# alan-turing-institute/mogp-emulator

Measured on AMD Instinct MI355X. Metric: GP fits/sec (+ fit+grad/s, predict pts/s), 64-output n=2000 d=10 on 1 MI355X, fp64, higher is better.
Workload: dtype f64

## Files before the change

### mogp_emulator_amd/csrc/kernels_mchol.hip

```cpp
#include <algorithm>
#include <cmath>
#include <cstdio>
#include <cstdlib>
#include <utility>
#include <vector>
#define MOGP_OPAQUE_TID 1
#include "launch.h"
#include "chol128_dev.h"
#include "trsm_dev.h"
#include "gemm_dev.h"

namespace mogp {

namespace {

constexpr int MC_LINE = 32;
constexpr int MC_ABORT = 0, MC_TIMEOUTS = 1;
constexpr int MC_HEADS = MC_LINE;
constexpr int MC_EMU0 = MC_LINE * 9;
constexpr int MC_AHEAD_BIT = 1 << 29;
constexpr int MC_PD = 4;
constexpr int MC_LDS_HDR = 4;

__device__ __forceinline__ unsigned ldu(const unsigned* p) { return __hip_atomic_load(p, __ATOMIC_RELAXED, __HIP_MEMORY_SCOPE_AGENT); }
__device__ __forceinline__ void stu(unsigned* p, unsigned x) { __hip_atomic_store(p, x, __ATOMIC_RELAXED, __HIP_MEMORY_SCOPE_AGENT); }
__device__ __forceinline__ void drain_stores() { asm volatile("s_waitcnt vmcnt(0)" ::: "memory"); }

#ifndef MOGP_MC_SCHED
#define MOGP_MC_SCHED 3
#endif
constexpr int MC_SCHED = MOGP_MC_SCHED;
template <int BM, int BN>
__device__ __forceinline__ void MC_GEMM(const double* __restrict__ Ag, int lda, const double* __restrict__ Bg, int ldb, int nk, v4d (&acc)[BM / 32][BN / 32],
                                        double* smem, int kmask) {
  mainloop_q<BM, BN, 2, 2, 2, MC_SCHED>(Ag, lda, Bg, ldb, nk, acc, smem, kmask);
}
constexpr size_t MC_GEMM_LDS = QCfg<64, 128>::SMEM_DOUBLES;

struct McCtx {
  unsigned* ctrl;
  int spin_limit;
  int* shi;
};

constexpr int MC_TRW = 30;
template <bool TRACE>
__device__ __forceinline__ void mc_stamp(unsigned long long* tr, int i) {
  if (TRACE && tr && threadIdx.x == 0) tr[i] = __builtin_amdgcn_s_memrealtime();
}

__device__ __forceinline__ int mc_wait_min4(const McCtx& cx, const unsigned* a, const unsigned* b, const unsigned* c, const unsigned* d, unsigned want,
                                            unsigned long long* waited = nullptr) {
  if (threadIdx.x == 0) {
    const unsigned long long w0 = waited ? __builtin_amdgcn_s_memrealtime() : 0ull;
    int res, spins = 0;
    for (;;) {
      unsigned m = ldu(a);
      const unsigned mb = ldu(b), mc = ldu(c), md = ldu(d);
      m = m < mb ? m : mb;
      m = m < mc ? m : mc;
      m = m < md ? m : md;
      if (m >= want) {
        res = (int)m;
        break;
      }
      ++spins;
      if (spins > cx.spin_limit) {
        stu(cx.ctrl + MC_ABORT, 1u);
        __hip_atomic_fetch_add(cx.ctrl + MC_TIMEOUTS, 1u, __ATOMIC_RELAXED, __HIP_MEMORY_SCOPE_AGENT);
        res = -1;
        break;
      }
      if ((spins & 31) == 0 && ldu(cx.ctrl + MC_ABORT) != 0u) {
        res = -1;
        break;
      }
      __builtin_amdgcn_s_sleep(1);
    }
    cx.shi[1] = res;
    if (waited) waited[9] += __builtin_amdgcn_s_memrealtime() - w0;
  }
  __syncthreads();
  const int r = cx.shi[1];
  __syncthreads();
  return r;
}

__device__ __forceinline__ int mc_wait_min3(const McCtx& cx, const unsigned* a, const unsigned* b, const unsigned* c, unsigned want,
                                            unsigned long long* waited = nullptr) {
  return mc_wait_min4(cx, a, b, c, c, want, waited);
}

struct PieceWait {
  const McCtx& cx;
  const unsigned *a, *b;
  unsigned base;
  int avail;
  unsigned long long* tr;
  __device__ __forceinline__ bool known(int j) const { return avail > j; }
  __device__ __forceinline__ bool operator()(int j) {
    if (avail > j) return true;
    const int m = mc_wait_min3(cx, a, b, b, base + (unsigned)j + 1u, tr);
    if (m < 0) return false;
    avail = m - (int)base;
    return true;
  }
};

}

template <bool TRACE, bool SOLO = false>
__global__ __launch_bounds__(256, SOLO ? 1 : 2) void mchol_kernel(BatchView v, unsigned* __restrict__ ctrl, const int* __restrict__ table, int ntasks,
                                                       int emu_stride, double* __restrict__ packs, int* __restrict__ info, int nq, int spin_limit,
                                                       unsigned long long* __restrict__ trace, int opts) {
  extern __shared__ __attribute__((aligned(16))) double smem[];
  int* shi = reinterpret_cast<int*>(smem);
  double* lds = smem + MC_LDS_HDR;
  McCtx cx{ctrl, spin_limit, shi};
  const int t = threadIdx.x;
  const int ld = v.LD;
  const int K = v.NP / 128, K2 = v.NP / 64;
  const int home = (int)blockIdx.x & (nq - 1);
  const int emus_q = v.nb / nq;
  const int total = ntasks * emus_q;
  const int gs = ((opts >> 12) & 0xff) ? ((opts >> 12) & 0xff) : emus_q;
  for (int qi = 0; qi < nq; ++qi) {
    const int q = (home + qi) & (nq - 1);
    unsigned* head = ctrl + MC_HEADS + q * MC_LINE;
    int next_tk = -1;
    auto draw_next = [&]() {
      if (t == 0 && next_tk < 0) next_tk = (int)__hip_atomic_fetch_add(head, 1u, __ATOMIC_RELAXED, __HIP_MEMORY_SCOPE_AGENT);
    };
    for (;;) {
      draw_next();
      if (t == 0) shi[0] = next_tk;
      __syncthreads();
      const int tk = shi[0];
      __syncthreads();
      if (tk >= total) break;
      next_tk = -1;
      const int per = ntasks * gs, grp = tk / per, rem = tk - grp * per;
      const int p = rem / gs, zl = grp * gs + (rem - p * gs);
      const int z = zl * nq + q;
      const int emu = __builtin_amdgcn_readfirstlane(v.idx ? v.idx[z] : z);
      const int word = table[p];
      const int type = (word >> 30) & 3, c = (word >> 15) & 0x3fff, r = word & 0x7fff;
      const bool listed_ahead = (word & MC_AHEAD_BIT) != 0;
      double* A = v.A + (size_t)emu * v.MS;
      unsigned* rowdone = ctrl + MC_EMU0 + (size_t)z * emu_stride;
      unsigned* diagcnt = rowdone + K2;
      unsigned* ddone = diagcnt + K;
      unsigned* rowprog = ddone + K;
      double* pk = packs + ((size_t)z * K + c) * PACK128_STRIDE;
      const int c0 = 128 * c;
      unsigned long long* tr = TRACE ? trace + ((size_t)z * ntasks + p) * MC_TRW : nullptr;
      if (TRACE && t == 0) {
        tr[6] = __builtin_amdgcn_s_getreg(6164) | ((unsigned long long)__builtin_amdgcn_s_getreg(((8 - 1) << 11) | (8 << 6) | 4) << 8);
        tr[7] = (unsigned)word | ((unsigned long long)tk << 32);
      }
      mc_stamp<TRACE>(tr, 0);
      if (type == 0) {
        mc_stamp<TRACE>(tr, 1);
        if (c > 1 && mc_wait_min3(cx, diagcnt + c, diagcnt + c, diagcnt + c, 3u, tr) < 0) return;
        auto inputs_seen = [&]() { mc_stamp<TRACE>(tr, 2); };
        if (c > 0) {
          PieceWait pw{cx, rowprog + 2 * c, rowprog + 2 * c + 1, 8u * (unsigned)(c - 1), 0, tr};
          if (!chol128_dev<true, true, true>(A + (size_t)c0 * ld + c0, ld, pk, info + emu, c0, lds, ddone + c, pw, inputs_seen)) return;
        } else {
          inputs_seen();
          chol128_dev<true, false, true>(A + (size_t)c0 * ld + c0, ld, pk, info + emu, c0, lds, ddone + c);
        }
        __builtin_amdgcn_s_setprio(0);
        drain_stores();
        __syncthreads();
        if (t == 0) stu(ddone + c, 8u);
        mc_stamp<TRACE>(tr, 5);
        continue;
      }
      if (type == 1) {
        const int ti = r > 0 ? 1 : 0, tj = r > 1 ? 1 : 0;
        const int gi0 = c0 + 64 * ti, gj0 = c0 + 64 * tj;
        __builtin_amdgcn_s_setprio(2);
        v4d acc[2][2];
        double* pcG = A + (size_t)(gi0 + (t >> 7) * 32 + ((t & 63) >> 4)) * ld + (gj0 + ((t >> 6) & 1) * 32 + (t & 15));
#pragma unroll
        for (int i = 0; i < 2; ++i)
#pragma unroll
          for (int j = 0; j < 2; ++j)
#pragma unroll
            for (int q = 0; q < 4; ++q) acc[i][j][q] = SOLO ? -pcG[(size_t)(i * 16 + 4 * q) * ld + j * 16] : 0.0;
        const int kend = c - 1;
        int kb = 0;
        while (kb < kend) {
          mc_stamp<TRACE>(tr, 1);
          int m = mc_wait_min3(cx, rowdone + 2 * c + ti, rowdone + 2 * c + tj, rowdone + 2 * c + tj, (unsigned)(kb + 1), tr);
          if (m < 0) return;
          mc_stamp<TRACE>(tr, 2);
          m = m < kend ? m : kend;
          MC_GEMM<64, 64>(A + (size_t)gi0 * ld + 128 * kb, ld, A + (size_t)gj0 * ld + 128 * kb, ld, 8 * (m - kb), acc, lds, -1);
          kb = m;
        }
        mc_stamp<TRACE>(tr, 3);
        draw_next();
        {
          double cv[2][2][4];
          if (!SOLO) {
#pragma unroll
            for (int i = 0; i < 2; ++i)
#pragma unroll
              for (int j = 0; j < 2; ++j)
#pragma unroll
                for (int q = 0; q < 4; ++q) cv[i][j][q] = pcG[(size_t)(i * 16 + 4 * q) * ld + j * 16];
          }
#pragma unroll
          for (int i = 0; i < 2; ++i)
#pragma unroll
            for (int j = 0; j < 2; ++j)
#pragma unroll
              for (int q = 0; q < 4; ++q)
                __hip_atomic_store(pcG + (size_t)(i * 16 + 4 * q) * ld + j * 16, SOLO ? -acc[i][j][q] : cv[i][j][q] - acc[i][j][q], __ATOMIC_RELAXED,
                                   __HIP_MEMORY_SCOPE_AGENT);
        }
        drain_stores();
        mc_stamp<TRACE>(tr, 4);
        __syncthreads();
        if (t == 0) __hip_atomic_fetch_add(diagcnt + c, 1u, __ATOMIC_RELAXED, __HIP_MEMORY_SCOPE_AGENT);
        mc_stamp<TRACE>(tr, 5);
        __builtin_amdgcn_s_setprio(0);
        continue;
      }
      const int r0 = 64 * r;
      const bool urgent = r < 2 * c + 4 + 2 * ((opts >> 8) & 3);
      if (urgent) __builtin_amdgcn_s_setprio(2);
      const int kend = c;
      if (kend > 0) {
        v4d acc[2][4];
        const double* pcT = A + (size_t)(r0 + (t >> 7) * 32 + ((t & 63) >> 4)) * ld + (c0 + ((t >> 6) & 1) * 64 + (t & 15));
#pragma unroll
        for (int i = 0; i < 2; ++i)
#pragma unroll
          for (int j = 0; j < 4; ++j)
#pragma unroll
            for (int q = 0; q < 4; ++q) acc[i][j][q] = SOLO ? -pcT[(size_t)(i * 16 + 4 * q) * ld + j * 16] : 0.0;
        auto finish_x = [&]() {
          if (SOLO) {
#pragma unroll
            for (int i = 0; i < 2; ++i)
#pragma unroll
              for (int j = 0; j < 4; ++j) acc[i][j] = -acc[i][j];
          } else {
            double cv[2][4][4];
#pragma unroll
            for (int i = 0; i < 2; ++i)
#pragma unroll
              for (int j = 0; j < 4; ++j)
#pragma unroll
                for (int q = 0; q < 4; ++q) cv[i][j][q] = pcT[(size_t)(i * 16 + 4 * q) * ld + j * 16];
#pragma unroll
            for (int i = 0; i < 2; ++i)
#pragma unroll
              for (int j = 0; j < 4; ++j)
#pragma unroll
                for (int q = 0; q < 4; ++q) acc[i][j][q] = cv[i][j][q] - acc[i][j][q];
          }
        };
        {
          int ks = 0;
          const int kse = 8 * kend;
          while (ks < kse) {
            mc_stamp<TRACE>(tr, 1);
            int have = mc_wait_min3(cx, rowprog + r, rowprog + 2 * c, rowprog + 2 * c + 1, (unsigned)(ks + MC_PD), tr);
            if (have < 0) return;
            mc_stamp<TRACE>(tr, 2);
            have = (have < kse ? have : kse) & ~(MC_PD - 1);
            MC_GEMM<64, 128>(A + (size_t)r0 * ld + 16 * ks, ld, A + (size_t)c0 * ld + 16 * ks, ld, have - ks, acc, lds,
                             (opts & 2) ? 3 : -1);
            ks = have;
          }
        }
        mc_stamp<TRACE>(tr, 3);
        if (!listed_ahead) draw_next();
        if (!urgent) {
          if (mc_wait_min3(cx, ddone + c, ddone + c, ddone + c, 8u, tr) < 0) return;
          TrsmSlabPre SP;
          trsm128_slab_request(pk, SP);
          finish_x();
          mc_stamp<TRACE>(tr, 4);
          mc_stamp<TRACE>(tr, 8);
          __builtin_amdgcn_s_setprio(1);
          trsm128_tile2_dev<true>(v, c0, r0, pk, emu, lds, acc, SP, TRACE ? tr + 10 : nullptr);
          drain_stores();
          mc_stamp<TRACE>(tr, 13);
          __syncthreads();
          if (t == 0) {
            stu(rowprog + r, 8u * (unsigned)(c + 1));
            stu(rowdone + r, (unsigned)(c + 1));
          }
          mc_stamp<TRACE>(tr, 5);
          __builtin_amdgcn_s_setprio(0);
          continue;
        }
        {
          finish_x();
          mc_stamp<TRACE>(tr, 4);
          bool first = true;
          auto wait = [&](int b) {
            const bool ok = mc_wait_min3(cx, ddone + c, ddone + c, ddone + c, (unsigned)(b + 1), tr) >= 0;
            if (first) mc_stamp<TRACE>(tr, 8);
            first = false;
            return ok;
          };
          auto pub = [&](int b) {
            if (t == 0) stu(rowprog + r, 8u * (unsigned)c + (unsigned)b + 1u);
          };
          const int prog = mc_wait_min3(cx, ddone + c, ddone + c, ddone + c, 0u);
          if (prog < 0) return;
          if (prog >= 8) {
            mc_stamp<TRACE>(tr, 8);
            trsm128_tile2_chain_dev<true, true>(v, c0, r0, pk, emu, lds, acc, TrsmNoWait(), pub);
          } else if (!trsm128_tile2_chain_dev<true, false>(v, c0, r0, pk, emu, lds, acc, wait, pub)) return;
          drain_stores();
          __syncthreads();
          if (t == 0) {
            stu(rowprog + r, 8u * (unsigned)(c + 1));
            stu(rowdone + r, (unsigned)(c + 1));
          }
          mc_stamp<TRACE>(tr, 5);
          __builtin_amdgcn_s_setprio(0);
          continue;
        }
      }
      if (urgent) {
        bool first = true;
        auto wait = [&](int b) {
          const bool ok = mc_wait_min3(cx, ddone + c, ddone + c, ddone + c, (unsigned)(b + 1), tr) >= 0;
          if (first) mc_stamp<TRACE>(tr, 8);
          first = false;
          return ok;
        };
        auto pub = [&](int b) {
          if (t == 0) stu(rowprog + r, 8u * (unsigned)c + (unsigned)b + 1u);
        };
        const int prog = mc_wait_min3(cx, ddone + c, ddone + c, ddone + c, 0u);
        if (prog < 0) return;
        if (prog >= 8) {
          mc_stamp<TRACE>(tr, 8);
          trsm128_lds_dev<true, true, false>(v, c0, r0, pk, emu, 0, lds, TrsmNoWait(), pub);
        } else if (!trsm128_lds_dev<true, false, true>(v, c0, r0, pk, emu, 0, lds, wait, pub)) return;
      } else {
        if (mc_wait_min3(cx, ddone + c, ddone + c, ddone + c, 8u, tr) < 0) return;
        mc_stamp<TRACE>(tr, 8);
        __builtin_amdgcn_s_setprio(1);
        trsm128_lds_dev<true, true>(v, c0, r0, pk, emu, 0, lds);
      }
      drain_stores();
      __syncthreads();
      if (t == 0) {
        stu(rowprog + r, 8u * (unsigned)(c + 1));
        stu(rowdone + r, (unsigned)(c + 1));
      }
      mc_stamp<TRACE>(tr, 5);
      __builtin_amdgcn_s_setprio(0);
    }
  }
}

std::vector<int> mchol_task_table(int NP, bool ahead) {
  const int K = NP / 128, K2 = NP / 64;
  auto word = [](int type, int c, int r) { return (int)(((unsigned)type << 30) | ((unsigned)c << 15) | (unsigned)r); };
  std::vector<std::pair<long, int>> keyed;
  const long M = 4L * K2 + 64;
  long slot = 0;
  int iter = -1;
  auto put = [&](int w, bool band) {
    const bool moved = band && ahead && iter >= 1;
    keyed.push_back({(long)((moved ? iter - 1 : iter) + 1) * M + (moved ? M / 2 : 0) + slot, moved ? (w | MC_AHEAD_BIT) : w});
    ++slot;
  };
  auto T = [&](int r, int c, bool band) {
    if (c < K && r < K2 && r >= 2 * c + 2) put(word(2, c, r), band);
  };
  put(word(0, 0, 0), false);
  T(2, 0, false);
  T(3, 0, false);
  T(4, 0, false);
  T(5, 0, false);
  for (int c = 0; c < K; ++c) {
    iter = c;
    slot = 0;
    if (c + 1 < K) put(word(0, c + 1, 0), false);
    T(2 * c + 4, c + 1, true);
    T(2 * c + 5, c + 1, true);
    if (c + 2 < K)
      for (int sub = 0; sub < 3; ++sub) put(word(1, c + 2, sub), false);
    T(2 * c + 6, c, true);
    T(2 * c + 7, c, true);
    T(2 * c + 6, c + 1, true);
    T(2 * c + 7, c + 1, true);
    for (int r = 2 * c + 8; r < K2; ++r) T(r, c, false);
  }
  std::stable_sort(keyed.begin(), keyed.end(), [](const std::pair<long, int>& a, const std::pair<long, int>& b) { return a.first < b.first; });
  std::vector<int> tb;
  for (auto& kw : keyed) tb.push_back(kw.second);
  return tb;
}

int mchol_emu_stride(int NP) { return (2 * (NP / 64) + 2 * (NP / 128) + MC_LINE - 1) / MC_LINE * MC_LINE; }
size_t mchol_ctrl_ints(int NP, int B) { return MC_EMU0 + (size_t)B * mchol_emu_stride(NP); }
size_t mchol_pack_doubles(int NP, int B) { return (size_t)B * (NP / 128) * PACK128_STRIDE; }

static double mchol_rho(int nb, int NP) {
  const double npd = NP;
  return ((double)nb * npd * npd * npd / 3.0 / 45e12) / ((npd / 128.0) * 55e-6);
}

void launch_mchol(const BatchView& v, unsigned* ctrl, size_t ctrl_ints, const int* tables, int ntasks, double* packs, int* info, int n_cu,
                  hipStream_t s, bool ctrl_zeroed) {
  static const int spin_limit = [] { const char* e = getenv("MOGP_MC_SPIN"); return e ? atoi(e) : (1 << 22); }();
  const double rho = mchol_rho(v.nb, v.NP);
  const double K16 = std::max(1.0, (v.NP / 128) / 16.0);
  const int per_cu = rho < 1.2 * std::pow(K16, 0.7) ? 1 : 2;

  if (!ctrl_zeroed) (void)hipMemsetAsync(ctrl, 0, ctrl_ints * sizeof(unsigned), s);
  const int nq = (v.nb % 8 == 0) ? 8 : 1;
  const size_t lds_need = MC_LDS_HDR + std::max<size_t>({(size_t)MC_GEMM_LDS, (size_t)TRSM128L_LDS, (size_t)C128_LDS_PRE_DOUBLES, (size_t)TRSM128T_LDS});
  const size_t lds_doubles = per_cu == 1 ? std::max<size_t>(lds_need, 10 * 1024 + 64) : lds_need;
  const int total = ntasks * v.nb;
  const int grid = std::min(per_cu * n_cu, total);
  const bool ahead = rho >= 0.2 && rho < 2.0 && 8 * (v.nb / nq) <= grid / nq;
  const int* table = tables + (ahead ? ntasks : 0);
  static const char* trace_file = getenv("MOGP_MC_TRACE");
  const size_t words = (size_t)total * MC_TRW;
  unsigned long long* dtr = nullptr;
  const int emus_q = v.nb / nq, wg_q = std::max(1, grid / nq);
  int gsz = 0;
  if (v.NP >= 2048)
    for (int g = 1; g < emus_q; ++g)
      if (emus_q % g == 0 && 4 * g * (v.NP / 64) >= 5 * wg_q) {
        gsz = g;
        break;
      }
  const int opts = ((rho < 1.0 ? 2 : 0) << 8) | (gsz << 12);
  if (trace_file) {
    if (hipMalloc(reinterpret_cast<void**>(&dtr), words * 8) != hipSuccess) {
      dtr = nullptr;
      fprintf(stderr, "libmogp_hip: MOGP_MC_TRACE: no device memory for %zu stamp words, this factorisation is not traced\n", words);
    }
  }
  if (trace_file && dtr) {
    (void)hipMemsetAsync(dtr, 0, words * 8, s);
    hipLaunchKernelGGL(mchol_kernel<true>, dim3(grid), dim3(256), lds_doubles * sizeof(double), s, v, ctrl, table, ntasks, mchol_emu_stride(v.NP), packs,
                       info, nq, spin_limit, dtr, opts);
    std::vector<unsigned long long> h(words);
    (void)hipStreamSynchronize(s);
    (void)hipMemcpy(h.data(), dtr, words * 8, hipMemcpyDeviceToHost);
    (void)hipFree(dtr);
    if (FILE* f = fopen(trace_file, "ab")) {
      const long long hdr[4] = {v.nb, ntasks, v.NP, grid + 1000000LL * MC_TRW};
      fwrite(hdr, sizeof(hdr), 1, f);
      fwrite(h.data(), 8, words, f);
      fclose(f);
    }
    return;
  }
  prof_begin("mchol", s);
  if (per_cu == 1)
    hipLaunchKernelGGL((mchol_kernel<false, true>), dim3(grid), dim3(256), lds_doubles * sizeof(double), s, v, ctrl, table, ntasks, mchol_emu_stride(v.NP), packs,
                     info, nq, spin_limit, (unsigned long long*)nullptr, opts);
  else
    hipLaunchKernelGGL(mchol_kernel<false>, dim3(grid), dim3(256), lds_doubles * sizeof(double), s, v, ctrl, table, ntasks, mchol_emu_stride(v.NP), packs,
                     info, nq, spin_limit, (unsigned long long*)nullptr, opts);
  const double n = v.n;
  prof_end("mchol", s, (double)v.nb * n * n * n / 3.0, (double)v.nb * 8.0 * n * n);
}

}
```

### mogp_emulator_amd/csrc/trsm_dev.h

```cpp
#pragma once
#include <type_traits>
#include "launch.h"
#include "chol128_dev.h"

namespace mogp {

typedef double v4d_t __attribute__((ext_vector_type(4)));
typedef double v2d_p __attribute__((ext_vector_type(2)));

constexpr int TL_PK = 112 * 16 + 256;
constexpr int TL_TS = 16 * 18;
constexpr int TRSM128L_LDS = 2 * TL_PK + 4 * 2 * TL_TS;

struct TrsmNoWait {
  __device__ __forceinline__ bool operator()(int) const { return true; }
};
struct TrsmNoPub {
  __device__ __forceinline__ void operator()(int) const {}
};
template <bool SC1_OUT = false, bool DEEP = false, bool PIPE = false, class WAIT = TrsmNoWait, class PUB = TrsmNoPub>
__device__ __forceinline__ bool trsm128_lds_dev(const BatchView& v, int c0, int r0, const double* __restrict__ pk, int emu, int rowblock,
                                                double* lds, WAIT wait = WAIT(), PUB pub = PUB()) {
  constexpr bool PUBLISH = (PIPE || DEEP) && !std::is_same<PUB, TrsmNoPub>::value;
  Sc1Buf ab;
  if (SC1_OUT) ab = sc1_buf(v.A + (size_t)emu * v.MS, (unsigned)(v.MS * sizeof(double)));
  const int ld = v.LD;
  const int t = mogp_tid(), lane = t & 63, wave = __builtin_amdgcn_readfirstlane(t >> 6);
  const int g = lane >> 4, i = lane & 15;
  double* slab = v.A + (size_t)emu * v.MS + (size_t)(r0 + rowblock * 64 + wave * 16) * ld + c0;
  double* pkb[2] = {lds, lds + TL_PK};
  double* tsb[2] = {lds + 2 * TL_PK + wave * 2 * TL_TS, lds + 2 * TL_PK + wave * 2 * TL_TS + TL_TS};
  const double* LT = pk + PACK128_LT;
  const int sr0 = lane >> 3, sp = (lane & 7) * 2;
  constexpr bool PRE_SLAB = DEEP || PIPE;
  v2d_p sl[PRE_SLAB ? 8 : 1][2];
  auto slab_request = [&](int b) {
    sl[PRE_SLAB ? b : 0][0] = *reinterpret_cast<const v2d_p*>(slab + (size_t)sr0 * ld + 16 * b + sp);
    sl[PRE_SLAB ? b : 0][1] = *reinterpret_cast<const v2d_p*>(slab + (size_t)(sr0 + 8) * ld + 16 * b + sp);
  };
  auto slab_deposit = [&](int b, double* ts) {
    *reinterpret_cast<v2d_p*>(ts + sr0 * 18 + sp) = sl[PRE_SLAB ? b : 0][0];
    *reinterpret_cast<v2d_p*>(ts + (sr0 + 8) * 18 + sp) = sl[PRE_SLAB ? b : 0][1];
  };
  v2d_p pr[DEEP ? 2 : 1][4], pinv[DEEP ? 2 : 1];
  auto pack_request = [&](int b) {
    const int u = DEEP ? (b & 1) : 0;
#pragma unroll
    for (int q = 0; q < 4; ++q) {
      const int ch = t + 256 * q;
      if (ch < 128 * b) pr[u][q] = *reinterpret_cast<const v2d_p*>(LT + (size_t)(ch >> 3) * 128 + 16 * b + (ch & 7) * 2);
    }
    if (t < 128) pinv[u] = *reinterpret_cast<const v2d_p*>(pk + PACK128_INV + b * 256 + 2 * t);
  };
  auto pack_deposit = [&](int b, double* img) {
    const int u = DEEP ? (b & 1) : 0;
#pragma unroll
    for (int q = 0; q < 4; ++q) {
      const int ch = t + 256 * q;
      if (ch < 128 * b) *reinterpret_cast<v2d_p*>(img + (ch >> 3) * 16 + (ch & 7) * 2) = pr[u][q];
    }
    if (t < 128) *reinterpret_cast<v2d_p*>(img + 112 * 16 + 2 * t) = pinv[u];
  };
  if (PIPE) {
#pragma unroll
    for (int b = 0; b < 8; ++b) slab_request(b);
    if (!wait(0)) return false;
    pack_request(0);
  } else {
    pack_request(0);
    if (DEEP) {
      pack_request(1);
#pragma unroll
      for (int b = 0; b < 8; ++b) slab_request(b);
    } else {
      slab_request(0);
    }
  }
  pack_deposit(0, pkb[0]);
  slab_deposit(0, tsb[0]);
  __syncthreads();
  v4d_t X[8];
#pragma unroll
  for (int b = 0; b < 8; ++b) {
    const double* img = pkb[b & 1];
    double* ts = tsb[b & 1];
    if (PIPE) {
    } else if (DEEP) {
      if (b + 2 < 8) pack_request(b + 2);
    } else if (b < 7) {
      pack_request(b + 1);
      slab_request(b + 1);
    }
    v4d_t T;
#pragma unroll
    for (int r = 0; r < 4; ++r) T[r] = ts[i * 18 + g + 4 * r];
#pragma unroll
    for (int a = 0; a < b; ++a)
#pragma unroll
      for (int r = 0; r < 4; ++r)
        T = __builtin_amdgcn_mfma_f64_16x16x4f64(-img[(16 * a + g + 4 * r) * 16 + i], X[a][r], T, 0, 0, 0);
    const double* inv = img + 112 * 16;
    X[b] = (v4d_t){0., 0., 0., 0.};
#pragma unroll
    for (int r = 0; r < 4; ++r) X[b] = __builtin_amdgcn_mfma_f64_16x16x4f64(inv[(g + 4 * r) * 16 + i], T[r], X[b], 0, 0, 0);
#pragma unroll
    for (int r = 0; r < 4; ++r) ts[i * 18 + g + 4 * r] = X[b][r];
    __builtin_amdgcn_wave_barrier();
    {
      const v2d_p o0 = *reinterpret_cast<const v2d_p*>(ts + sr0 * 18 + sp);
      const v2d_p o1 = *reinterpret_cast<const v2d_p*>(ts + (sr0 + 8) * 18 + sp);
      st16<SC1_OUT>(ab, slab + (size_t)sr0 * ld + 16 * b + sp, o0);
      st16<SC1_OUT>(ab, slab + (size_t)(sr0 + 8) * ld + 16 * b + sp, o1);
    }
    if (PUBLISH && b < 7) {
      asm volatile("s_waitcnt vmcnt(0)" ::: "memory");
      __syncthreads();
      pub(b);
    }
    if (b < 7) {
      if (PIPE) {
        if (!wait(b + 1)) return false;
        pack_request(b + 1);
      }
      pack_deposit(b + 1, pkb[(b + 1) & 1]);
      slab_deposit(b + 1, tsb[(b + 1) & 1]);
    }
    __syncthreads();
  }
  return true;
}

constexpr int TRSM128T_LDS = 2 * TL_PK + 16 * TL_TS;
struct TrsmSlabPre {
  v2d_p pr[2][4], pinv[2];
};
__device__ __forceinline__ void trsm128_slab_request(const double* __restrict__ pk, TrsmSlabPre& P) {
  const int t = mogp_tid();
  const double* LT = pk + PACK128_LT;
#pragma unroll
  for (int b = 0; b < 2; ++b) {
#pragma unroll
    for (int q = 0; q < 4; ++q) {
      const int ch = t + 256 * q;
      if (ch < 128 * (7 - b)) P.pr[b][q] = *reinterpret_cast<const v2d_p*>(LT + (size_t)(16 * b + ((ch >> 3) & 15)) * 128 + 16 * (b + 1 + (ch >> 7)) + (ch & 7) * 2);
    }
    if (t < 128) P.pinv[b] = *reinterpret_cast<const v2d_p*>(pk + PACK128_INV + b * 256 + 2 * t);
  }
}

constexpr int TL_TS17 = 16 * 17;
static_assert(32 * TL_TS17 <= TRSM128T_LDS, "whole-tile stage must fit the LDS of the half-tile form");
template <bool SC1_OUT>
__device__ __forceinline__ void trsm128_tile2_dev(const BatchView& v, int c0, int r0, const double* __restrict__ pk, int emu, double* lds,
                                                  const v4d_t (&x)[2][4], TrsmSlabPre& P, unsigned long long* stamps = nullptr) {
  Sc1Buf ab;
  if (SC1_OUT) ab = sc1_buf(v.A + (size_t)emu * v.MS, (unsigned)(v.MS * sizeof(double)));
  const int ld = v.LD;
  const int t = mogp_tid(), lane = t & 63, wave = __builtin_amdgcn_readfirstlane(t >> 6);
  const int g = lane >> 4, i = lane & 15;
  const int wr = wave >> 1, wc = wave & 1;
  double* slab = v.A + (size_t)emu * v.MS + (size_t)(r0 + wave * 16) * ld + c0;
  double* pkb[2] = {lds, lds + TL_PK};
  double* ts = lds + 2 * TL_PK + wave * TL_TS;
  const double* LT = pk + PACK128_LT;
  const int sr0 = lane >> 3, sp = (lane & 7) * 2;
  auto pack_request = [&](int b) {
    const int u = b & 1;
#pragma unroll
    for (int q = 0; q < 4; ++q) {
      const int ch = t + 256 * q;
      if (ch < 128 * (7 - b))
        P.pr[u][q] = *reinterpret_cast<const v2d_p*>(LT + (size_t)(16 * b + ((ch >> 3) & 15)) * 128 + 16 * (b + 1 + (ch >> 7)) + (ch & 7) * 2);
    }
    if (t < 128) P.pinv[u] = *reinterpret_cast<const v2d_p*>(pk + PACK128_INV + b * 256 + 2 * t);
  };
  auto pack_deposit = [&](int b, double* img) {
    const int u = b & 1;
#pragma unroll
    for (int q = 0; q < 4; ++q) {
      const int ch = t + 256 * q;
      if (ch < 128 * (7 - b)) *reinterpret_cast<v2d_p*>(img + ((b + 1 + (ch >> 7)) * 16 + ((ch >> 3) & 15)) * 16 + (ch & 7) * 2) = P.pr[u][q];
    }
    if (t < 128) *reinterpret_cast<v2d_p*>(img + 2 * t) = P.pinv[u];
  };
#pragma unroll
  for (int ii = 0; ii < 2; ++ii)
#pragma unroll
    for (int j = 0; j < 4; ++j)
#pragma unroll
      for (int q = 0; q < 4; ++q) lds[((2 * wr + ii) * 8 + 4 * wc + j) * TL_TS17 + (g + 4 * q) * 17 + i] = x[ii][j][q];
  __syncthreads();
  v4d_t T[8];
#pragma unroll
  for (int b = 0; b < 8; ++b)
#pragma unroll
    for (int r = 0; r < 4; ++r) T[b][r] = lds[(wave * 8 + b) * TL_TS17 + i * 17 + g + 4 * r];
  __syncthreads();
  pack_deposit(0, pkb[0]);
  __syncthreads();
  if (stamps && t == 0) stamps[0] = __builtin_amdgcn_s_memrealtime();
  v4d_t X[8];
#pragma unroll
  for (int b = 0; b < 8; ++b) {
    const double* img = pkb[b & 1];
    if (b + 2 < 8) pack_request(b + 2);
    X[b] = (v4d_t){0., 0., 0., 0.};
#pragma unroll
    for (int r = 0; r < 4; ++r) X[b] = __builtin_amdgcn_mfma_f64_16x16x4f64(img[(g + 4 * r) * 16 + i], T[b][r], X[b], 0, 0, 0);
#pragma unroll
    for (int c = b + 1; c < 8; ++c)
#pragma unroll
      for (int r = 0; r < 4; ++r) T[c] = __builtin_amdgcn_mfma_f64_16x16x4f64(-img[(16 * c + g + 4 * r) * 16 + i], X[b][r], T[c], 0, 0, 0);
    __builtin_amdgcn_wave_barrier();
#pragma unroll
    for (int r = 0; r < 4; ++r) ts[i * 18 + g + 4 * r] = X[b][r];
    __builtin_amdgcn_wave_barrier();
    if (stamps && t == 0) stamps[4 + 2 * b] = __builtin_amdgcn_s_memrealtime();
    {
      const v2d_p o0 = *reinterpret_cast<const v2d_p*>(ts + sr0 * 18 + sp);
      const v2d_p o1 = *reinterpret_cast<const v2d_p*>(ts + (sr0 + 8) * 18 + sp);
      st16<SC1_OUT>(ab, slab + (size_t)sr0 * ld + 16 * b + sp, o0);
      st16<SC1_OUT>(ab, slab + (size_t)(sr0 + 8) * ld + 16 * b + sp, o1);
    }
    __builtin_amdgcn_wave_barrier();
    if (b == 3 && stamps && t == 0) stamps[1] = __builtin_amdgcn_s_memrealtime();
    if (b < 7) pack_deposit(b + 1, pkb[(b + 1) & 1]);
    __syncthreads();
    if (stamps && t == 0) stamps[5 + 2 * b] = __builtin_amdgcn_s_memrealtime();
  }
  if (stamps && t == 0) stamps[2] = __builtin_amdgcn_s_memrealtime();
}

template <bool SC1_OUT, bool LATE, class WAIT, class PUB>
__device__ __forceinline__ bool trsm128_tile2_chain_dev(const BatchView& v, int c0, int r0, const double* __restrict__ pk, int emu, double* lds,
                                                        const v4d_t (&x)[2][4], WAIT wait, PUB pub) {
  Sc1Buf ab;
  if (SC1_OUT) ab = sc1_buf(v.A + (size_t)emu * v.MS, (unsigned)(v.MS * sizeof(double)));
  const int ld = v.LD;
  const int t = mogp_tid(), lane = t & 63, wave = __builtin_amdgcn_readfirstlane(t >> 6);
  const int g = lane >> 4, i = lane & 15;
  const int wr = wave >> 1, wc = wave & 1;
  double* slab = v.A + (size_t)emu * v.MS + (size_t)(r0 + wave * 16) * ld + c0;
  double* pkb[2] = {lds, lds + TL_PK};
  double* ts = lds + 2 * TL_PK + wave * TL_TS;
  const double* LT = pk + PACK128_LT;
  const int sr0 = lane >> 3, sp = (lane & 7) * 2;
  v2d_p pr[2][4], pinv[2];
  auto pack_request = [&](int b) {
    const int u = b & 1;
#pragma unroll
    for (int q = 0; q < 4; ++q) {
      const int ch = t + 256 * q;
      if (ch < 128 * b) pr[u][q] = *reinterpret_cast<const v2d_p*>(LT + (size_t)(ch >> 3) * 128 + 16 * b + (ch & 7) * 2);
    }
    if (t < 128) pinv[u] = *reinterpret_cast<const v2d_p*>(pk + PACK128_INV + b * 256 + 2 * t);
  };
  auto pack_deposit = [&](int b, double* img) {
    const int u = b & 1;
#pragma unroll
    for (int q = 0; q < 4; ++q) {
      const int ch = t + 256 * q;
      if (ch < 128 * b) *reinterpret_cast<v2d_p*>(img + (ch >> 3) * 16 + (ch & 7) * 2) = pr[u][q];
    }
    if (t < 128) *reinterpret_cast<v2d_p*>(img + 112 * 16 + 2 * t) = pinv[u];
  };
  auto rows_request = [&](int b) {
    const int u = b & 1;
#pragma unroll
    for (int q = 0; q < 4; ++q) {
      const int ch = t + 256 * q;
      if (ch < 128 * b) pr[u][q] = *reinterpret_cast<const v2d_p*>(LT + (size_t)(ch >> 3) * 128 + 16 * b + (ch & 7) * 2);
    }
  };
  auto rows_deposit = [&](int b, double* img) {
    const int u = b & 1;
#pragma unroll
    for (int q = 0; q < 4; ++q) {
      const int ch = t + 256 * q;
      if (ch < 128 * b) *reinterpret_cast<v2d_p*>(img + (ch >> 3) * 16 + (ch & 7) * 2) = pr[u][q];
    }
  };
#pragma unroll
  for (int ii = 0; ii < 2; ++ii)
#pragma unroll
    for (int j = 0; j < 4; ++j)
#pragma unroll
      for (int q = 0; q < 4; ++q) lds[((2 * wr + ii) * 8 + 4 * wc + j) * TL_TS17 + (g + 4 * q) * 17 + i] = x[ii][j][q];
  __syncthreads();
  v4d_t T[8];
#pragma unroll
  for (int b = 0; b < 8; ++b)
#pragma unroll
    for (int r = 0; r < 4; ++r) T[b][r] = lds[(wave * 8 + b) * TL_TS17 + i * 17 + g + 4 * r];
  if (LATE) {
    pack_request(0);
    pack_request(1);
    __syncthreads();
    pack_deposit(0, pkb[0]);
  }
  __syncthreads();
  v4d_t X[8];
#pragma unroll
  for (int b = 0; b < 8; ++b) {
    const double* img = pkb[b & 1];
    if (LATE && b + 2 < 8) pack_request(b + 2);
    v4d_t Tb = T[b];
    if (b > 0) {
      double an[4], ac[4];
#pragma unroll
      for (int r = 0; r < 4; ++r) an[r] = img[(g + 4 * r) * 16 + i];
#pragma unroll
      for (int a = 0; a < b; ++a) {
#pragma unroll
        for (int r = 0; r < 4; ++r) ac[r] = an[r];
        if (a + 1 < b) {
#pragma unroll
          for (int r = 0; r < 4; ++r) an[r] = img[(16 * (a + 1) + g + 4 * r) * 16 + i];
        }
        __builtin_amdgcn_sched_barrier(0);
#pragma unroll
        for (int r = 0; r < 4; ++r) Tb = __builtin_amdgcn_mfma_f64_16x16x4f64(ac[r], X[a][r], Tb, 0, 0, 0);
        __builtin_amdgcn_sched_barrier(0);
      }
    }
    double invr[4];
    if (LATE) {
      const double* inv = img + 112 * 16;
#pragma unroll
      for (int r = 0; r < 4; ++r) invr[r] = inv[(g + 4 * r) * 16 + i];
    } else {
      if (!wait(b)) return false;
#pragma unroll
      for (int r = 0; r < 4; ++r) invr[r] = pk[PACK128_INV + b * 256 + (g + 4 * r) * 16 + i];
      if (b + 1 < 8) rows_request(b + 1);
    }
    X[b] = (v4d_t){0., 0., 0., 0.};
#pragma unroll
    for (int r = 0; r < 4; ++r) X[b] = __builtin_amdgcn_mfma_f64_16x16x4f64(invr[r], Tb[r], X[b], 0, 0, 0);
    __builtin_amdgcn_wave_barrier();
#pragma unroll
    for (int r = 0; r < 4; ++r) ts[i * 18 + g + 4 * r] = X[b][r];
    X[b] = -X[b];
    __builtin_amdgcn_wave_barrier();
    {
      const v2d_p o0 = *reinterpret_cast<const v2d_p*>(ts + sr0 * 18 + sp);
      const v2d_p o1 = *reinterpret_cast<const v2d_p*>(ts + (sr0 + 8) * 18 + sp);
      st16<SC1_OUT>(ab, slab + (size_t)sr0 * ld + 16 * b + sp, o0);
      st16<SC1_OUT>(ab, slab + (size_t)(sr0 + 8) * ld + 16 * b + sp, o1);
    }
    if (b < 7) {
      asm volatile("s_waitcnt vmcnt(0)" ::: "memory");
      __syncthreads();
      pub(b);
      if (LATE) pack_deposit(b + 1, pkb[(b + 1) & 1]);
      else rows_deposit(b + 1, pkb[(b + 1) & 1]);
    }
    __syncthreads();
  }
  return true;
}

template <bool SC1_OUT>
__device__ __forceinline__ void trsm128_tile_dev(const BatchView& v, int c0, int r0, const double* __restrict__ pk, int emu, double* lds,
                                                 const v4d_t (&x)[2][4], unsigned long long* stamps = nullptr) {
  Sc1Buf ab;
  if (SC1_OUT) ab = sc1_buf(v.A + (size_t)emu * v.MS, (unsigned)(v.MS * sizeof(double)));
  const int ld = v.LD;
  const int t = mogp_tid(), lane = t & 63, wave = __builtin_amdgcn_readfirstlane(t >> 6);
  const int g = lane >> 4, i = lane & 15;
  const int wr = wave >> 1, wc = wave & 1;
  double* slab = v.A + (size_t)emu * v.MS + (size_t)(r0 + wave * 16) * ld + c0;
  double* pkb[2] = {lds, lds + TL_PK};
  double* stage = lds + 2 * TL_PK;
  const double* LT = pk + PACK128_LT;
  const int sr0 = lane >> 3, sp = (lane & 7) * 2;
  v2d_p pr[2][4], pinv[2];
  auto pack_request = [&](int b) {
    const int u = b & 1;
#pragma unroll
    for (int q = 0; q < 4; ++q) {
      const int ch = t + 256 * q;
      if (ch < 128 * b) pr[u][q] = *reinterpret_cast<const v2d_p*>(LT + (size_t)(ch >> 3) * 128 + 16 * b + (ch & 7) * 2);
    }
    if (t < 128) pinv[u] = *reinterpret_cast<const v2d_p*>(pk + PACK128_INV + b * 256 + 2 * t);
  };
  auto pack_deposit = [&](int b, double* img) {
    const int u = b & 1;
#pragma unroll
    for (int q = 0; q < 4; ++q) {
      const int ch = t + 256 * q;
      if (ch < 128 * b) *reinterpret_cast<v2d_p*>(img + (ch >> 3) * 16 + (ch & 7) * 2) = pr[u][q];
    }
    if (t < 128) *reinterpret_cast<v2d_p*>(img + 112 * 16 + 2 * t) = pinv[u];
  };
  auto tile_deposit = [&](int h) {
    if (wc == h) {
#pragma unroll
      for (int ii = 0; ii < 2; ++ii)
#pragma unroll
        for (int j = 0; j < 4; ++j)
#pragma unroll
          for (int q = 0; q < 4; ++q) stage[((2 * wr + ii) * 4 + j) * TL_TS + (g + 4 * q) * 18 + i] = x[ii][j][q];
    }
  };
  pack_request(0);
  pack_request(1);
  tile_deposit(0);
  pack_deposit(0, pkb[0]);
  __syncthreads();
  if (stamps && t == 0) stamps[0] = __builtin_amdgcn_s_memrealtime();
  v4d_t X[8];
#pragma unroll
  for (int b = 0; b < 8; ++b) {
    const double* img = pkb[b & 1];
    double* ts = stage + (wave * 4 + (b & 3)) * TL_TS;
    if (b + 2 < 8) pack_request(b + 2);
    v4d_t T;
#pragma unroll
    for (int r = 0; r < 4; ++r) T[r] = ts[i * 18 + g + 4 * r];
#pragma unroll
    for (int a = 0; a < b; ++a)
#pragma unroll
      for (int r = 0; r < 4; ++r) T = __builtin_amdgcn_mfma_f64_16x16x4f64(-img[(16 * a + g + 4 * r) * 16 + i], X[a][r], T, 0, 0, 0);
    const double* inv = img + 112 * 16;
    X[b] = (v4d_t){0., 0., 0., 0.};
#pragma unroll
    for (int r = 0; r < 4; ++r) X[b] = __builtin_amdgcn_mfma_f64_16x16x4f64(inv[(g + 4 * r) * 16 + i], T[r], X[b], 0, 0, 0);
    __builtin_amdgcn_wave_barrier();
#pragma unroll
    for (int r = 0; r < 4; ++r) ts[i * 18 + g + 4 * r] = X[b][r];
    __builtin_amdgcn_wave_barrier();
    if (stamps && t == 0) stamps[4 + 2 * b] = __builtin_amdgcn_s_memrealtime();
    {
      const v2d_p o0 = *reinterpret_cast<const v2d_p*>(ts + sr0 * 18 + sp);
      const v2d_p o1 = *reinterpret_cast<const v2d_p*>(ts + (sr0 + 8) * 18 + sp);
      st16<SC1_OUT>(ab, slab + (size_t)sr0 * ld + 16 * b + sp, o0);
      st16<SC1_OUT>(ab, slab + (size_t)(sr0 + 8) * ld + 16 * b + sp, o1);
    }
    if (b == 3) {
      __syncthreads();
      if (stamps && t == 0) stamps[1] = __builtin_amdgcn_s_memrealtime();
      tile_deposit(1);
    }
    if (b < 7) pack_deposit(b + 1, pkb[(b + 1) & 1]);
    __syncthreads();
    if (stamps && t == 0) stamps[5 + 2 * b] = __builtin_amdgcn_s_memrealtime();
  }
  if (stamps && t == 0) stamps[2] = __builtin_amdgcn_s_memrealtime();
}

}
```

Baseline: 16340.

## Invert diagonal Cholesky block once and apply panel solves as triangular multiplies

Result: slower. 15750 (-3.6%).

```diff
diff --git a/mogp_emulator_amd/csrc/kernels_mchol.hip b/mogp_emulator_amd/csrc/kernels_mchol.hip
--- a/mogp_emulator_amd/csrc/kernels_mchol.hip
+++ b/mogp_emulator_amd/csrc/kernels_mchol.hip
@@ -174,6 +174,12 @@
         drain_stores();
         __syncthreads();
         if (t == 0) stu(ddone + c, 8u);
+        if (!SOLO && c > 0) {
+          trinv128_dev(pk, lds);
+          drain_stores();
+          __syncthreads();
+          if (t == 0) stu(ddone + c, 9u);
+        }
         mc_stamp<TRACE>(tr, 5);
         continue;
       }
@@ -281,14 +287,16 @@
         mc_stamp<TRACE>(tr, 3);
         if (!listed_ahead) draw_next();
         if (!urgent) {
-          if (mc_wait_min3(cx, ddone + c, ddone + c, ddone + c, 8u, tr) < 0) return;
+          if (mc_wait_min3(cx, ddone + c, ddone + c, ddone + c, SOLO ? 8u : 9u, tr) < 0) return;
           TrsmSlabPre SP;
-          trsm128_slab_request(pk, SP);
+          if (SOLO) trsm128_slab_request(pk, SP);
+          else trmm128_slab_request(pk, SP);
           finish_x();
           mc_stamp<TRACE>(tr, 4);
           mc_stamp<TRACE>(tr, 8);
           __builtin_amdgcn_s_setprio(1);
-          trsm128_tile2_dev<true>(v, c0, r0, pk, emu, lds, acc, SP, TRACE ? tr + 10 : nullptr);
+          if (SOLO) trsm128_tile2_dev<true>(v, c0, r0, pk, emu, lds, acc, SP, TRACE ? tr + 10 : nullptr);
+          else trmm128_tile2_dev<true>(v, c0, r0, pk, emu, lds, acc, SP, TRACE ? tr + 10 : nullptr);
           drain_stores();
           mc_stamp<TRACE>(tr, 13);
           __syncthreads();
diff --git a/mogp_emulator_amd/csrc/trsm_dev.h b/mogp_emulator_amd/csrc/trsm_dev.h
--- a/mogp_emulator_amd/csrc/trsm_dev.h
+++ b/mogp_emulator_amd/csrc/trsm_dev.h
@@ -231,6 +231,184 @@
   if (stamps && t == 0) stamps[2] = __builtin_amdgcn_s_memrealtime();
 }
 
+constexpr int TW_LD = 130;
+constexpr int TW_IMG = 16 * TW_LD + 256;
+static_assert(2 * TW_IMG + 4 * TL_TS <= TRSM128T_LDS, "images and the four stages of the way out must fit the LDS of the tile solve");
+__device__ __forceinline__ void trmm128_image_request(const double* __restrict__ pk, int b, v2d_p (&pr)[4], v2d_p& pinv) {
+  const int t = mogp_tid();
+  const int w8 = b > 0 ? 8 * b : 1;
+#pragma unroll
+  for (int q = 0; q < 4; ++q) {
+    const int ch = t + 256 * q;
+    if (ch < 128 * b) {
+      const int i = ch / w8, kc = ch - i * w8;
+      pr[q] = *reinterpret_cast<const v2d_p*>(pk + PACK128_LT + (size_t)(16 * b + i) * 128 + 2 * kc);
+    }
+  }
+  if (t < 128) pinv = *reinterpret_cast<const v2d_p*>(pk + PACK128_INV + b * 256 + 2 * t);
+}
+__device__ __forceinline__ void trmm128_image_deposit(double* img, int b, const v2d_p (&pr)[4], const v2d_p& pinv) {
+  const int t = mogp_tid();
+  const int w8 = b > 0 ? 8 * b : 1;
+#pragma unroll
+  for (int q = 0; q < 4; ++q) {
+    const int ch = t + 256 * q;
+    if (ch < 128 * b) {
+      const int i = ch / w8, kc = ch - i * w8;
+      *reinterpret_cast<v2d_p*>(img + i * TW_LD + 2 * kc) = pr[q];
+    }
+  }
+  if (t < 128) *reinterpret_cast<v2d_p*>(img + 16 * TW_LD + 2 * t) = pinv;
+}
+__device__ __forceinline__ void trmm128_slab_request(const double* __restrict__ pk, TrsmSlabPre& P) {
+  trmm128_image_request(pk, 7, P.pr[0], P.pinv[0]);
+  trmm128_image_request(pk, 6, P.pr[1], P.pinv[1]);
+}
+template <bool SC1_OUT>
+__device__ __forceinline__ void trmm128_tile2_dev(const BatchView& v, int c0, int r0, const double* __restrict__ pk, int emu, double* lds,
+                                                  const v4d_t (&x)[2][4], TrsmSlabPre& P, unsigned long long* stamps = nullptr) {
+  Sc1Buf ab;
+  if (SC1_OUT) ab = sc1_buf(v.A + (size_t)emu * v.MS, (unsigned)(v.MS * sizeof(double)));
+  const int ld = v.LD;
+  const int t = mogp_tid(), lane = t & 63, wave = __builtin_amdgcn_readfirstlane(t >> 6);
+  const int g = lane >> 4, i = lane & 15;
+  const int wr = wave >> 1, wc = wave & 1;
+  double* slab = v.A + (size_t)emu * v.MS + (size_t)(r0 + wave * 16) * ld + c0;
+  double* pkb[2] = {lds, lds + TW_IMG};
+  double* ts = lds + 2 * TW_IMG + wave * TL_TS;
+  const int sr0 = lane >> 3, sp = (lane & 7) * 2;
+#pragma unroll
+  for (int ii = 0; ii < 2; ++ii)
+#pragma unroll
+    for (int j = 0; j < 4; ++j)
+#pragma unroll
+      for (int q = 0; q < 4; ++q) lds[((2 * wr + ii) * 8 + 4 * wc + j) * TL_TS17 + (g + 4 * q) * 17 + i] = x[ii][j][q];
+  __syncthreads();
+  v4d_t T[8];
+#pragma unroll
+  for (int b = 0; b < 8; ++b)
+#pragma unroll
+    for (int r = 0; r < 4; ++r) T[b][r] = lds[(wave * 8 + b) * TL_TS17 + i * 17 + g + 4 * r];
+  __syncthreads();
+  trmm128_image_deposit(pkb[0], 7, P.pr[0], P.pinv[0]);
+  __syncthreads();
+  if (stamps && t == 0) stamps[0] = __builtin_amdgcn_s_memrealtime();
+#pragma unroll
+  for (int s = 0; s < 8; ++s) {
+    const int b = 7 - s;
+    const double* img = pkb[s & 1];
+    if (s + 2 < 8) trmm128_image_request(pk, b - 2, P.pr[s & 1], P.pinv[s & 1]);
+    v4d_t S[4];
+#pragma unroll
+    for (int r = 0; r < 4; ++r) S[r] = (v4d_t){0., 0., 0., 0.};
+#pragma unroll
+    for (int a = 0; a < b; ++a)
+#pragma unroll
+      for (int r = 0; r < 4; ++r) S[r] = __builtin_amdgcn_mfma_f64_16x16x4f64(img[i * TW_LD + 16 * a + g + 4 * r], T[a][r], S[r], 0, 0, 0);
+    const double* inv = img + 16 * TW_LD;
+#pragma unroll
+    for (int r = 0; r < 4; ++r) S[r] = __builtin_amdgcn_mfma_f64_16x16x4f64(inv[(g + 4 * r) * 16 + i], T[b][r], S[r], 0, 0, 0);
+    const v4d_t X = (S[0] + S[1]) + (S[2] + S[3]);
+    __builtin_amdgcn_wave_barrier();
+#pragma unroll
+    for (int r = 0; r < 4; ++r) ts[i * 18 + g + 4 * r] = X[r];
+    __builtin_amdgcn_wave_barrier();
+    if (stamps && t == 0) stamps[4 + 2 * s] = __builtin_amdgcn_s_memrealtime();
+    {
+      const v2d_p o0 = *reinterpret_cast<const v2d_p*>(ts + sr0 * 18 + sp);
+      const v2d_p o1 = *reinterpret_cast<const v2d_p*>(ts + (sr0 + 8) * 18 + sp);
+      st16<SC1_OUT>(ab, slab + (size_t)sr0 * ld + 16 * b + sp, o0);
+      st16<SC1_OUT>(ab, slab + (size_t)(sr0 + 8) * ld + 16 * b + sp, o1);
+    }
+    __builtin_amdgcn_wave_barrier();
+    if (s == 3 && stamps && t == 0) stamps[1] = __builtin_amdgcn_s_memrealtime();
+    if (s < 7) trmm128_image_deposit(pkb[(s + 1) & 1], b - 1, P.pr[(s + 1) & 1], P.pinv[(s + 1) & 1]);
+    __syncthreads();
+    if (stamps && t == 0) stamps[5 + 2 * s] = __builtin_amdgcn_s_memrealtime();
+  }
+  if (stamps && t == 0) stamps[2] = __builtin_amdgcn_s_memrealtime();
+}
+
+__device__ __forceinline__ void trinv128_dev(double* __restrict__ pk, double* lds) {
+  const Sc1Buf pb = sc1_buf(pk, PACK128_STRIDE * sizeof(double));
+  const int t = mogp_tid(), lane = t & 63, wave = __builtin_amdgcn_readfirstlane(t >> 6);
+  const int g = lane >> 4, i = lane & 15;
+  const int a1 = wave, a2 = 7 - wave;
+  double* pkb[2] = {lds, lds + TL_PK};
+  const double* LT = pk + PACK128_LT;
+  v2d_p pr[2][4], pinv[2];
+  auto pack_request = [&](int b) {
+    const int u = b & 1;
+#pragma unroll
+    for (int q = 0; q < 4; ++q) {
+      const int ch = t + 256 * q;
+      if (ch < 128 * b) pr[u][q] = *reinterpret_cast<const v2d_p*>(LT + (size_t)(ch >> 3) * 128 + 16 * b + (ch & 7) * 2);
+    }
+    if (t < 128) pinv[u] = *reinterpret_cast<const v2d_p*>(pk + PACK128_INV + b * 256 + 2 * t);
+  };
+  auto pack_deposit = [&](int b, double* img) {
+    const int u = b & 1;
+#pragma unroll
+    for (int q = 0; q < 4; ++q) {
+      const int ch = t + 256 * q;
+      if (ch < 128 * b) *reinterpret_cast<v2d_p*>(img + (ch >> 3) * 16 + (ch & 7) * 2) = pr[u][q];
+    }
+    if (t < 128) *reinterpret_cast<v2d_p*>(img + 112 * 16 + 2 * t) = pinv[u];
+  };
+  typedef unsigned int u2_t __attribute__((ext_vector_type(2)));
+  auto put = [&](int b, int a, const v4d_t& X) {
+#pragma unroll
+    for (int r = 0; r < 4; ++r) {
+      const double xr = X[r];
+      __builtin_amdgcn_raw_buffer_store_b64(__builtin_bit_cast(u2_t, xr), pb.rs,
+                                            (unsigned)((PACK128_LT + (16 * b + g + 4 * r) * 128 + 16 * a + i) * sizeof(double)), 0, 16);
+    }
+  };
+  v4d_t ident;
+#pragma unroll
+  for (int r = 0; r < 4; ++r) ident[r] = (g + 4 * r == i) ? 1.0 : 0.0;
+  const v4d_t zero4 = {0., 0., 0., 0.};
+  pack_request(0);
+  pack_request(1);
+  pack_deposit(0, pkb[0]);
+  __syncthreads();
+  v4d_t X1[8], X2[8];
+#pragma unroll
+  for (int k = 0; k < 8; ++k) X1[k] = X2[k] = zero4;
+#pragma unroll
+  for (int b = 0; b < 8; ++b) {
+    const double* img = pkb[b & 1];
+    const double* inv = img + 112 * 16;
+    if (b + 2 < 8) pack_request(b + 2);
+    if (b >= a1) {
+      v4d_t T = b == a1 ? ident : zero4;
+#pragma unroll
+      for (int k = 0; k < b; ++k)
+        if (k >= a1) {
+#pragma unroll
+          for (int r = 0; r < 4; ++r) T = __builtin_amdgcn_mfma_f64_16x16x4f64(-img[(16 * k + g + 4 * r) * 16 + i], X1[k][r], T, 0, 0, 0);
+        }
+#pragma unroll
+      for (int r = 0; r < 4; ++r) X1[b] = __builtin_amdgcn_mfma_f64_16x16x4f64(inv[(g + 4 * r) * 16 + i], T[r], X1[b], 0, 0, 0);
+      if (b > a1) put(b, a1, X1[b]);
+    }
+    if (b >= 4 && b >= a2) {
+      v4d_t T = b == a2 ? ident : zero4;
+#pragma unroll
+      for (int k = 4; k < b; ++k)
+        if (k >= a2) {
+#pragma unroll
+          for (int r = 0; r < 4; ++r) T = __builtin_amdgcn_mfma_f64_16x16x4f64(-img[(16 * k + g + 4 * r) * 16 + i], X2[k][r], T, 0, 0, 0);
+        }
+#pragma unroll
+      for (int r = 0; r < 4; ++r) X2[b] = __builtin_amdgcn_mfma_f64_16x16x4f64(inv[(g + 4 * r) * 16 + i], T[r], X2[b], 0, 0, 0);
+      if (b > a2) put(b, a2, X2[b]);
+    }
+    if (b < 7) pack_deposit(b + 1, pkb[(b + 1) & 1]);
+    __syncthreads();
+  }
+}
+
 template <bool SC1_OUT, bool LATE, class WAIT, class PUB>
 __device__ __forceinline__ bool trsm128_tile2_chain_dev(const BatchView& v, int c0, int r0, const double* __restrict__ pk, int emu, double* lds,
                                                         const v4d_t (&x)[2][4], WAIT wait, PUB pub) {
```
